# apache/horaedb

Hardware: NVIDIA H100
Metric: scanned rows/s (higher is better)
Workload: dtype f64

## Files before the change

### horaedb_b200/csrc/fused_scan.cu

```cuda
#include "fused_scan.h"

#include "block_scan.h"

#include <algorithm>
#include <cstddef>
#include <cstdlib>

namespace horae {
namespace fused {

namespace {

constexpr int MAXC = 8;
constexpr int kWarpsPerCta = 8;

struct alignas(16) FRec {
  uint32_t item, local;
  uint64_t gkey;
  int64_t bucket;
  uint64_t count;
  double sum, mn, mx;
  uint64_t _pad;
};

struct VSeg { const uint8_t* base1; uint32_t n0, _pad; };

enum : uint32_t { K_RAW64 = 0, K_U32 = 1, K_I32 = 2, K_F32 = 3 };
inline uint32_t kind_of(uint32_t t) {
  return (t == T_U64 || t == T_I64 || t == T_F64) ? K_RAW64 : (t == T_F32 ? K_F32 : ((t == T_I8 || t == T_I16 || t == T_I32) ? K_I32 : K_U32));
}
constexpr uint64_t kI32KeyLo = (1ull << 63) - (1ull << 31), kI32KeyHi = (1ull << 63) + (1ull << 31) - 1;

struct FParams {
  const SstDev* ssts;
  const RgSel* sel;
  const uint32_t* d_nsel;
  const uint8_t* const* bases;
  uint32_t split;
  uint32_t pcol[MAX_PREDS], pcls[MAX_PREDS];
  uint32_t pbloom[MAX_PREDS];
  uint64_t phash[MAX_PREDS];
  int nslots;
  uint32_t col[MAXC], kind[MAXC], cls[MAXC];
  int npk;
  int has_group, has_ts, value_slot, global_mode;
  int hot_slot[kHot];
  uint64_t hot_flip[kHot], hot_lo[kHot], hot_span[kHot];
  int hot_haspred[kHot];
  int npred;
  int pslot[MAX_PREDS];
  uint32_t pop[MAX_PREDS];
  uint64_t plit[MAX_PREDS];
  int64_t window_ms;
  const uint8_t* scratch;
  uint64_t scratch_stride;
  int region[MAXC];
  int value_stored;
  int gate_bits;
  int gate_slot;
  uint64_t bits_off;
  VSeg* vseg;
  FRec* rec;
  uint32_t rec_cap;
  uint32_t* item_cnt;
  unsigned int* work;
  unsigned long long* counters;
  int* err;
};

__device__ __forceinline__ uint64_t ld_bytes8(const uint8_t* p) {
  uintptr_t a = reinterpret_cast<uintptr_t>(p);
  uint32_t sh = uint32_t(a & 7) * 8;
  const uint64_t* q = reinterpret_cast<const uint64_t*>(a & ~uintptr_t(7));
  uint64_t lo = __ldg(q), hi = __ldg(q + 1);
  return (lo >> sh) | ((hi << 1) << (63 - sh));
}
__device__ __forceinline__ uint32_t ld32u(const uint8_t* p) { return uint32_t(ld_bytes8(p)); }

__device__ __forceinline__ uint64_t widen_kind(uint64_t raw, uint32_t kind) {
  uint32_t r = uint32_t(raw);
  uint64_t v = raw;
  v = kind == K_U32 ? uint64_t(r) : v;
  v = kind == K_I32 ? uint64_t(int64_t(int32_t(r))) : v;
  v = kind == K_F32 ? uint64_t(__double_as_longlong(double(__uint_as_float(r)))) : v;
  return v;
}
__device__ __forceinline__ uint64_t load_kind(const uint8_t* base, uint32_t kind, uint32_t row) {
  return widen_kind(ld_bytes8(base + size_t(row) * (kind == K_RAW64 ? 8u : 4u)), kind);
}

__device__ __forceinline__ uint32_t literal_header(const uint8_t* p, uint32_t* len) {
  const uint32_t t = __ldg(p);
  uint32_t l = t >> 2, hdr = 1;
  if (l >= 60) {
    const uint32_t nb = l - 59;
    l = 0;
    for (uint32_t i = 0; i < nb; i++) l |= uint32_t(__ldg(p + 1 + i)) << (8 * i);
    hdr = 1 + nb;
  }
  *len = l + 1;
  return hdr;
}

__device__ __forceinline__ const uint8_t* slot_base_chase(const FParams& P, uint32_t si, int s) {
  RgSel rs = P.sel[si];
  SstDev sst = P.ssts[rs.sst];
  ChunkDev cd = sst.chunks[size_t(rs.rg) * sst.ncols + P.col[s]];
  PageDev pg = sst.pages[cd.first_page];
  const uint8_t* body = sst.bytes + pg.payload_off;
  const bool is_value = P.value_stored && s == P.value_slot;
  if (cd.codec == 1) {
    if (is_value && cd.stored) {
      const uint8_t* p = body;
      while (__ldg(p) & 0x80) p++;
      p++;
      uint32_t len0 = 0, len1 = 0;
      const uint32_t h0 = literal_header(p, &len0);
      const uint8_t* lit0 = p + h0;
      const uint32_t prefix = cd.optional ? 4 + ld32u(lit0) : 0;
      const uint32_t w = P.kind[s] == K_RAW64 ? 8u : 4u;
      VSeg v;
      v.n0 = (len0 - prefix) / w;
      v._pad = 0;
      v.base1 = lit0 + prefix;
      if (lit0 + len0 < body + pg.comp_size) v.base1 = lit0 + len0 + literal_header(lit0 + len0, &len1);
      P.vseg[si] = v;
      return lit0 + prefix;
    }
    body = P.scratch + rs.scratch_off + uint64_t(P.region[s]) * P.scratch_stride;
  }
  if (cd.optional && s != P.gate_slot) {
    uint32_t lv = ld32u(body);
    if (lv > pg.uncomp_size) { lv = 0; atomicExch(P.err, 202); }
    body += 4 + lv;
  }
  if (is_value) { VSeg v; v.base1 = body; v.n0 = rs.num_rows; v._pad = 0; P.vseg[si] = v; }
  return body;
}
__device__ __forceinline__ const uint8_t* slot_base(const FParams& P, uint32_t si, int s) { return P.bases[size_t(si) * MAXC + s]; }
__device__ __noinline__ uint64_t fetch_val(const FParams& P, uint32_t si, int s, uint32_t row) {
  return load_kind(slot_base(P, si, s), P.kind[s], row);
}

struct Bucket { int64_t start, lo, hi; };
__device__ __noinline__ Bucket bucket_range(int64_t ts, int64_t w) {
  constexpr int64_t kMin = INT64_MIN, kMax = INT64_MAX;
  const int64_t r = w - 1;
  Bucket b;
  b.start = ts / w * w;
  if (b.start > 0) { b.lo = b.start; b.hi = b.start > kMax - r ? kMax : b.start + r; }
  else if (b.start < 0) { b.lo = b.start < kMin + r ? kMin : b.start - r; b.hi = b.start; }
  else { b.lo = -r; b.hi = r; }
  return b;
}

__device__ __noinline__ bool later_alive_dup(const FParams& P, uint32_t si, uint32_t row) {
  uint64_t pk[MAX_PK];
  for (int k = 0; k < P.npk; k++) pk[k] = fetch_val(P, si, k, row);
  uint32_t nrows = P.sel[si].num_rows;
  uint32_t r = row + 1;
  for (;;) {
    if (r >= nrows) {
      si++;
      if (si >= *P.d_nsel) return false;
      nrows = P.sel[si].num_rows;
      r = 0;
      if (nrows == 0) continue;
    }
    for (int k = 0; k < P.npk; k++)
      if (fetch_val(P, si, k, r) != pk[k]) return false;
    bool ok = true;
    if (P.gate_slot >= 0) {
      const uint32_t* gb = reinterpret_cast<const uint32_t*>(P.scratch + P.sel[si].scratch_off + P.bits_off);
      ok = (gb[r >> 5] >> (r & 31)) & 1u;
    }
    for (int p = 0; p < P.npred && ok; p++)
      if (P.pslot[p] != P.gate_slot) ok = op_holds(cmp_widened(fetch_val(P, si, P.pslot[p], r), P.plit[p], P.cls[P.pslot[p]]), P.pop[p]);
    if (ok) return true;
    r++;
  }
}

__device__ __forceinline__ uint64_t shfl64(uint64_t v, int src) {
  uint32_t lo = __shfl_sync(0xffffffffu, uint32_t(v), src);
  uint32_t hi = __shfl_sync(0xffffffffu, uint32_t(v >> 32), src);
  return (uint64_t(hi) << 32) | lo;
}
__device__ __forceinline__ double shfl_xor_d(double v, int m) {
  uint64_t b = uint64_t(__double_as_longlong(v));
  uint32_t lo = __shfl_xor_sync(0xffffffffu, uint32_t(b), m);
  uint32_t hi = __shfl_xor_sync(0xffffffffu, uint32_t(b >> 32), m);
  return __longlong_as_double((long long)((uint64_t(hi) << 32) | lo));
}

struct Acc {
  bool open;
  uint64_t g;
  int64_t bstart, blo, bhi;
  uint64_t cnt;
  double sum, mn, mx;
};

__device__ __noinline__ void emit(const FParams& P, const Acc& a, uint32_t item, uint32_t local, uint32_t* slots) {
  if (slots[0] == slots[1]) { slots[0] = atomicAdd(&P.work[1], 32u); slots[1] = slots[0] + 32u; }
  unsigned int slot = slots[0]++;
  if (slot < P.rec_cap) {
    FRec r;
    r.item = item; r.local = local; r.gkey = a.g; r.bucket = a.bstart; r.count = a.cnt; r.sum = a.sum; r.mn = a.mn; r.mx = a.mx; r._pad = 0;
    P.rec[slot] = r;
  } else atomicExch(P.err, 201);
}

struct FileDev {
  const RgCol* rgcol;
  const uint32_t* rg_rows;
  uint32_t rg_base, nrg, ncols, _pad;
  const uint8_t* bytes;
};

__global__ void __launch_bounds__(256) slot_bases_kernel(const __grid_constant__ FParams P, const uint8_t** __restrict__ bases) {
  const uint32_t idx = blockIdx.x * blockDim.x + threadIdx.x;
  const uint32_t si = idx / MAXC;
  const int s = int(idx % MAXC);
  if (si >= *P.d_nsel || s >= P.nslots) return;
  bases[idx] = slot_base_chase(P, si, s);
}

template <bool W4>
__global__ void __launch_bounds__(256, 8) gate_rg_kernel(const __grid_constant__ FParams P, RgSel* __restrict__ sel, int gate_slot, uint64_t flip,
                                                      uint64_t lo, uint64_t span, uint8_t* __restrict__ flags) {
  constexpr int kRows = W4 ? 8 : 4;
  __shared__ uint32_t s_last;
  __shared__ const uint8_t* s_base[256];
  const uint32_t nsel = *P.d_nsel;
  const int lane = threadIdx.x & 31;
  for (uint32_t k0 = 0; blockIdx.x + k0 * gridDim.x < nsel; k0 += 256) {
    {
      const uint32_t si = blockIdx.x + (k0 + threadIdx.x) * gridDim.x;
      if (si < nsel) s_base[threadIdx.x] = slot_base_chase(P, si, gate_slot);
    }
    for (uint32_t k = 0; k < 256; k++) {
      const uint32_t si = blockIdx.x + (k0 + k) * gridDim.x;
      if (si >= nsel) break;
      if (threadIdx.x == 0) s_last = 0;
      __syncthreads();
      const uint8_t* base = s_base[k];
      const RgSel rs = sel[si];
      const uint32_t nrows = rs.num_rows;
      uint32_t* bits = P.gate_bits ? reinterpret_cast<uint32_t*>(const_cast<uint8_t*>(P.scratch) + rs.scratch_off + P.bits_off) : nullptr;
      const bool aligned = (reinterpret_cast<uintptr_t>(base) & (W4 ? 3 : 7)) == 0;
      uint32_t last = 0;
      const uint32_t nw = (nrows + 31) >> 5;
      for (uint32_t i0 = 0; i0 < nw * 32; i0 += kRows * 256) {
        uint64_t v[kRows];
#pragma unroll
        for (int u = 0; u < kRows; u++) {
          const uint32_t i = i0 + u * 256 + threadIdx.x;
          v[u] = 0;
          if (i < nrows) {
            if (W4) v[u] = aligned ? __ldg(reinterpret_cast<const uint32_t*>(base) + i) : ld32u(base + size_t(i) * 4);
            else v[u] = aligned ? __ldg(reinterpret_cast<const unsigned long long*>(base) + i) : ld_bytes8(base + size_t(i) * 8);
          }
        }
#pragma unroll
        for (int u = 0; u < kRows; u++) {
          const uint32_t i = i0 + u * 256 + threadIdx.x;
          const bool pass = i < nrows && (W4 ? (uint32_t(v[u]) ^ uint32_t(flip)) - uint32_t(lo) <= uint32_t(span) : (v[u] ^ flip) - lo <= span);
          if (pass) last = i + 1;
          const uint32_t b = __ballot_sync(0xffffffffu, pass);
          if (bits && lane == 0 && (i >> 5) < nw) bits[i >> 5] = b;
        }
      }
      for (int d = 16; d > 0; d >>= 1) { const uint32_t o = __shfl_down_sync(0xffffffffu, last, d); last = o > last ? o : last; }
      if (lane == 0 && last) atomicMax(&s_last, last);
      __syncthreads();
      if (threadIdx.x == 0) {
        const uint32_t l = s_last;
        flags[si] = l ? 1 : 0;
        sel[si].out_row = l ? (l + 1 < nrows ? l + 1 : nrows) : 0;
      }
    }
    __syncthreads();
  }
}

__global__ void __launch_bounds__(1024) compact_sel_kernel(const RgSel* __restrict__ in, const uint8_t* __restrict__ flags, uint32_t* d_nsel,
                                                           RgSel* __restrict__ out, uint32_t* __restrict__ lpt) {
  __shared__ uint32_t s_w[1024 / 32 + 1];
  __shared__ uint32_t s_bin[1024];
  __shared__ uint32_t s_max;
  const uint32_t n = *d_nsel;
  const uint32_t per = (n + 1023u) / 1024u;
  const uint32_t lo = threadIdx.x * per;
  const uint32_t hi = lo + per < n ? lo + per : n;
  uint32_t cnt = 0;
  for (uint32_t i = lo; i < hi; i++) cnt += flags[i] != 0;
  s_bin[threadIdx.x] = 0;
  if (threadIdx.x == 0) s_max = 0;
  uint32_t m;
  uint32_t pos = block_excl_scan<1024>(cnt, &m, s_w);
  uint32_t mx = 0;
  for (uint32_t i = lo; i < hi; i++)
    if (flags[i]) { out[pos++] = in[i]; mx = in[i].out_row > mx ? in[i].out_row : mx; }
  if (lpt) {
    if (mx) atomicMax(&s_max, mx);
    __syncthreads();
    int shift = 0;
    while ((s_max >> shift) > 1023u) shift++;
    const uint32_t per2 = (m + 1023u) / 1024u;
    const uint32_t lo2 = threadIdx.x * per2, hi2 = lo2 + per2 < m ? lo2 + per2 : m;
    for (uint32_t i = lo2; i < hi2; i++) atomicAdd(&s_bin[1023u - (out[i].out_row >> shift)], 1u);
    __syncthreads();
    uint32_t nbin;
    const uint32_t start = block_excl_scan<1024>(s_bin[threadIdx.x], &nbin, s_w);
    s_bin[threadIdx.x] = start;
    __syncthreads();
    for (uint32_t i = lo2; i < hi2; i++) lpt[atomicAdd(&s_bin[1023u - (out[i].out_row >> shift)], 1u)] = i;
  }
  __syncthreads();
  if (threadIdx.x == 0) *d_nsel = m;
}

__global__ void __launch_bounds__(256) prune_rgs_kernel(const __grid_constant__ FParams P, const FileDev* __restrict__ files, int nfiles,
                                                        uint32_t total_rgs, int prune, uint32_t* __restrict__ keep_rows) {
  const uint32_t idx = blockIdx.x * blockDim.x + threadIdx.x;
  if (idx >= total_rgs) return;
  uint32_t f = 0;
  while (f + 1 < uint32_t(nfiles) && idx >= files[f + 1].rg_base) f++;
  const FileDev fd = files[f];
  const uint32_t rg = idx - fd.rg_base;
  const uint32_t rows = fd.rg_rows[rg];
  uint32_t keep = rows > 0;
  if (keep && prune) {
    const RgCol* rc = fd.rgcol + size_t(rg) * fd.ncols;
    for (int p = 0; p < P.npred && keep; p++) {
      const RgCol c = rc[P.pcol[p]];
      if (c.null_all) { keep = 0; break; }
      if (c.has_minmax && !minmax_may_match(c.mn, c.mx, P.plit[p], P.pop[p], P.pcls[p])) keep = 0;
      else if ((prune & 2) && P.pbloom[p] && c.bloom_blocks && !bloom::may_contain(fd.bytes + c.bloom_off, c.bloom_blocks, P.phash[p])) keep = 0;
    }
  }
  keep_rows[idx] = keep ? rows : 0;
}

__global__ void __launch_bounds__(1024) select_rgs_kernel(const FileDev* __restrict__ files, int nfiles, uint32_t total_rgs,
                                                          const uint32_t* keep_rows, RgSel* __restrict__ sel, uint32_t* d_nsel,
                                                          unsigned long long* counters, uint32_t smem_words, uint64_t scratch_per_rg) {
  extern __shared__ uint32_t s_keep[];
  __shared__ uint32_t s_w[1024 / 32 + 1];
  if (smem_words) {
    for (uint32_t i = threadIdx.x; i < total_rgs; i += 1024) s_keep[i] = keep_rows[i];
    __syncthreads();
    keep_rows = s_keep;
  }
  const uint32_t per = (total_rgs + 1023u) / 1024u;
  const uint32_t lo = threadIdx.x * per;
  const uint32_t hi = lo + per < total_rgs ? lo + per : total_rgs;
  uint32_t cnt = 0;
  unsigned long long rows_sel = 0;
  for (uint32_t i = lo; i < hi; i++) { const uint32_t r = keep_rows[i]; cnt += r > 0; rows_sel += r; }
  uint32_t nsel;
  uint32_t pos = block_excl_scan<1024>(cnt, &nsel, s_w);
  if (cnt) {
    uint32_t f = 0;
    for (uint32_t i = lo; i < hi; i++) {
      const uint32_t rows = keep_rows[i];
      if (rows == 0) continue;
      while (f + 1 < uint32_t(nfiles) && i >= files[f + 1].rg_base) f++;
      RgSel r;
      r.sst = f; r.rg = i - files[f].rg_base; r.out_row = 0; r.num_rows = rows; r.scratch_off = uint64_t(pos) * scratch_per_rg;
      sel[pos++] = r;
    }
  }
  for (int d = 16; d > 0; d >>= 1) rows_sel += __shfl_down_sync(0xffffffffu, rows_sel, d);
  if ((threadIdx.x & 31) == 0 && rows_sel) atomicAdd(&counters[2], rows_sel);
  if (threadIdx.x == 0) *d_nsel = nsel;
}

struct KeyRef { uint64_t g; int64_t lo, hi; };

__device__ __forceinline__ uint64_t pack_pos(uint32_t si, uint32_t row) { return (uint64_t(si) << 32) | row; }

template <bool HAS_TS>
struct BoundSearch {
  uint32_t j, si, row, L, H, ans;
  KeyRef k;
  const uint8_t *b0, *b1;
  bool done, found;

  __device__ __forceinline__ void finish(uint64_t* adj, uint64_t v, int lane) { if (lane == 0) adj[j] = v; done = true; }

  __device__ __forceinline__ void open_rg(const FParams& P) {
    b0 = P.has_group ? slot_base(P, si, 0) : nullptr;
    b1 = HAS_TS ? slot_base(P, si, 1) : nullptr;
    L = row;
    H = P.sel[si].num_rows;
    found = false;
    ans = H;
  }

  __device__ __forceinline__ void init(const FParams& P, uint32_t jj, uint32_t nsel, uint32_t nitems, uint64_t* adj, int lane) {
    j = jj;
    done = false;
    if (j > nitems) { done = true; return; }
    if (j == nitems) { finish(adj, pack_pos(nsel, 0), lane); return; }
    si = j / P.split;
    const uint32_t w = j % P.split;
    const uint32_t n = P.sel[si].num_rows;
    const uint32_t sr = (((n + P.split - 1) / P.split) + 31u) & ~31u;
    row = w * sr;
    if (row >= n) { si++; row = 0; }
    if (si >= nsel) { finish(adj, pack_pos(nsel, 0), lane); return; }
    if (P.global_mode || (si == 0 && row == 0)) { finish(adj, pack_pos(si, row), lane); return; }
    uint32_t psi = si, prow = row;
    if (prow == 0) { psi--; prow = P.sel[psi].num_rows - 1; } else prow--;
    k.g = P.has_group ? fetch_val(P, psi, 0, prow) : 0;
    k.lo = 0; k.hi = 0;
    if (HAS_TS) { Bucket b = bucket_range(int64_t(fetch_val(P, psi, 1, prow)), P.window_ms); k.lo = b.lo; k.hi = b.hi; }
    open_rg(P);
  }

  __device__ __forceinline__ uint32_t probe_pos(int lane, uint32_t* step) const {
    const uint32_t span = H - L;
    *step = (span + 31) / 32;
    uint32_t p = L + (uint32_t(lane) + 1) * *step - 1;
    return p >= H ? H - 1 : p;
  }

  __device__ __forceinline__ void advance(const FParams& P, unsigned m, uint32_t step, uint32_t nsel, uint64_t* adj, int lane) {
    if (m == 0) L = H;
    else {
      const int f = __ffs(m) - 1;
      uint32_t pf = L + (uint32_t(f) + 1) * step - 1;
      if (pf >= H) pf = H - 1;
      found = true;
      ans = pf;
      if (step == 1) L = H;
      else { L = L + uint32_t(f) * step; H = pf; }
    }
    if (L >= H) {
      if (found) { finish(adj, pack_pos(si, ans), lane); return; }
      si++;
      row = 0;
      if (si >= nsel) { finish(adj, pack_pos(nsel, 0), lane); return; }
      open_rg(P);
    }
  }
};

constexpr int kBoundsPerWarp = 4;

template <bool HAS_TS>
__global__ void __launch_bounds__(256) item_bounds_kernel(const __grid_constant__ FParams P, uint64_t* __restrict__ adj) {
  const int lane = threadIdx.x & 31;
  const uint32_t nsel = *P.d_nsel;
  const uint32_t nitems = nsel * P.split;
  const uint32_t warp = (blockIdx.x * blockDim.x + threadIdx.x) >> 5;
  BoundSearch<HAS_TS> bs[kBoundsPerWarp];
#pragma unroll
  for (int i = 0; i < kBoundsPerWarp; i++) bs[i].init(P, warp * kBoundsPerWarp + i, nsel, nitems, adj, lane);
  for (;;) {
    bool any = false;
    uint32_t step[kBoundsPerWarp];
    uint64_t v0[kBoundsPerWarp], v1[kBoundsPerWarp];
#pragma unroll
    for (int i = 0; i < kBoundsPerWarp; i++) {
      v0[i] = 0; v1[i] = 0; step[i] = 1;
      if (!bs[i].done) {
        any = true;
        const uint32_t p = bs[i].probe_pos(lane, &step[i]);
        if (P.has_group) v0[i] = load_kind(bs[i].b0, P.kind[0], p);
        if (HAS_TS) v1[i] = load_kind(bs[i].b1, P.kind[1], p);
      }
    }
    if (!any) break;
#pragma unroll
    for (int i = 0; i < kBoundsPerWarp; i++) {
      if (!bs[i].done) {
        bool ne = (P.has_group && v0[i] != bs[i].k.g) || (HAS_TS && (int64_t(v1[i]) < bs[i].k.lo || int64_t(v1[i]) > bs[i].k.hi));
        const unsigned m = __ballot_sync(0xffffffffu, ne);
        bs[i].advance(P, m, step[i], nsel, adj, lane);
      }
    }
  }
}

__device__ __forceinline__ double seq_sum_slice(double sum, unsigned keep_mask, bool keep, double v, double* s_vals, int lane) {
  if (__popc(keep_mask) >= 8) {
    __syncwarp();
    s_vals[lane] = keep ? v : 0.0;
    __syncwarp();
#pragma unroll
    for (int l = 0; l < 32; l++) sum += s_vals[l];
    return sum;
  }
  uint64_t vb = uint64_t(__double_as_longlong(v));
  while (keep_mask) {
    int l = __ffs(keep_mask) - 1;
    keep_mask &= keep_mask - 1;
    sum += __longlong_as_double((long long)shfl64(vb, l));
  }
  return sum;
}

template <bool HAS_TS>
__device__ __noinline__ void walk_slice(const FParams& P, Acc& acc, uint32_t& local, uint32_t item, unsigned keep_mask, bool keep, uint64_t g,
                                        int64_t ts, double v, double* s_vals, uint32_t* slots, int lane) {
  const double kInf = __longlong_as_double(0x7ff0000000000000LL);
  const bool has_val = P.value_slot >= 0;
  bool ext = keep && acc.open && (!P.has_group || g == acc.g) && (!HAS_TS || (ts >= acc.blo && ts <= acc.bhi));
  if (__ballot_sync(0xffffffffu, ext) == keep_mask) {
    acc.cnt += __popc(keep_mask);
    if (has_val) {
      const bool num = keep && v == v;
      double mn = num ? v : kInf, mx = num ? v : -kInf;
#pragma unroll
      for (int m = 1; m < 32; m <<= 1) {
        const double a = shfl_xor_d(mn, m), b = shfl_xor_d(mx, m);
        const bool later = (lane & m) != 0;
        mn = (later ? a <= mn : a < mn) ? a : mn;
        mx = (later ? b >= mx : b > mx) ? b : mx;
      }
      acc.mn = mn < acc.mn ? mn : acc.mn;
      acc.mx = mx > acc.mx ? mx : acc.mx;
      acc.sum = seq_sum_slice(acc.sum, keep_mask, keep, v, s_vals, lane);
    }
    return;
  }
  uint64_t vb = uint64_t(__double_as_longlong(v));
  while (keep_mask) {
    int l = __ffs(keep_mask) - 1;
    keep_mask &= keep_mask - 1;
    uint64_t kg = P.has_group ? shfl64(g, l) : 0;
    int64_t kt = HAS_TS ? int64_t(shfl64(uint64_t(ts), l)) : 0;
    if (!acc.open || kg != acc.g || (HAS_TS && (kt < acc.blo || kt > acc.bhi))) {
      if (acc.open) { if (lane == 0) emit(P, acc, item, local, slots); local++; }
      acc.open = true; acc.g = kg; acc.cnt = 0; acc.sum = 0.0; acc.mn = kInf; acc.mx = -kInf;
      if (HAS_TS) { Bucket b = bucket_range(kt, P.window_ms); acc.bstart = b.start; acc.blo = b.lo; acc.bhi = b.hi; }
      else { acc.bstart = 0; acc.blo = 0; acc.bhi = 0; }
    }
    acc.cnt++;
    if (has_val) {
      double x = __longlong_as_double((long long)shfl64(vb, l));
      acc.sum += x;
      if (acc.cnt == 1 || x < acc.mn) acc.mn = x;
      if (acc.cnt == 1 || x > acc.mx) acc.mx = x;
    }
  }
}

__device__ __forceinline__ double to_double_kind(uint64_t raw, uint32_t kind, uint32_t cls) {
  uint64_t wv = widen_kind(raw, kind);
  return cls == C_FLOAT ? __longlong_as_double((long long)wv) : (cls == C_SIGNED ? double(int64_t(wv)) : double(wv));
}

__device__ __forceinline__ uint64_t ld8(const uint8_t* q, uint32_t sh, uint32_t i) {
  const uint64_t* p = reinterpret_cast<const uint64_t*>(q) + i;
  uint64_t lo = __ldg(p), hi = __ldg(p + 1);
  uint32_t w0 = uint32_t(lo), w1 = uint32_t(lo >> 32), w2 = uint32_t(hi), w3 = uint32_t(hi >> 32);
  const bool up = (sh & 32u) != 0;
  const uint32_t s = sh & 31u;
  uint32_t a = up ? w1 : w0, b = up ? w2 : w1, c = up ? w3 : w2;
  return (uint64_t(__funnelshift_r(b, c, s)) << 32) | __funnelshift_r(a, b, s);
}
__device__ __forceinline__ uint32_t ld4(const uint8_t* q, uint32_t sh, uint32_t i) {
  const uint32_t* p = reinterpret_cast<const uint32_t*>(q) + i;
  uint32_t lo = __ldg(p), hi = __ldg(p + 1);
  return __funnelshift_r(lo, hi, sh);
// ... 648 lines not shown
  CU_TRY(d_sel.alloc(size_t(total_rgs + 1) * sizeof(RgSel), s));
  CU_TRY(d_keep.alloc(size_t(total_rgs + 1) * sizeof(uint32_t), s));
  CU_TRY(d_bsum.alloc(1024 * sizeof(uint32_t), s));
  CU_TRY(d_bases.alloc(size_t(total_rgs + 1) * MAXC * sizeof(uint8_t*), s));
  if (value_stored) CU_TRY(d_vseg.alloc(size_t(total_rgs + 1) * sizeof(VSeg), s));
  if (need_snappy()) {
    CU_TRY(d_sel2.alloc(size_t(total_rgs + 1) * sizeof(RgSel), s));
    CU_TRY(d_gflags.alloc(size_t(total_rgs) + 16, s));
    CU_TRY(d_lpt.alloc(size_t(total_rgs + 1) * sizeof(uint32_t), s));
    CU_TRY(d_scratch.alloc(size_t(total_rgs) * size_t(scratch_per_rg) + 256, s));
  }
  CU_TRY(out->alloc(bound, s));
  return HG_OK;
}

int FusedPlan::make_params() {
  std::vector<SstDev> sd(files.size());
  std::vector<FileDev> fdv(files.size());
  uint32_t rgb = 0;
  for (size_t i = 0; i < files.size(); i++) {
    SstResident* f = files[i];
    sd[i] = SstDev{f->d_bytes, f->d_pages, f->d_chunks, uint32_t(f->meta.ncols), uint32_t(f->meta.rgs.size())};
    fdv[i] = FileDev{f->d_rgcol, f->d_rg_rows, rgb, uint32_t(f->rg_rows.size()), uint32_t(f->meta.ncols), 0, f->d_bytes};
    rgb += uint32_t(f->rg_rows.size());
  }
  CU_TRY(d_ssts.alloc(sd.size() * sizeof(SstDev), e->stream));
  CU_TRY(d_files.alloc(fdv.size() * sizeof(FileDev), e->stream));
  int urc = stage_upload(e, d_ssts.p, sd.data(), sd.size() * sizeof(SstDev));
  if (!urc) urc = stage_upload(e, d_files.p, fdv.data(), fdv.size() * sizeof(FileDev));
  if (urc) return urc;

  std::memset(&P, 0, sizeof(P));
  P.ssts = d_ssts.as<SstDev>();
  P.sel = d_sel.as<RgSel>();
  P.d_nsel = &work->nsel;
  P.bases = d_bases.as<const uint8_t*>();
  P.split = split;
  P.nslots = int(S.slots.size());
  for (size_t i = 0; i < S.slots.size(); i++) {
    uint32_t t = schema->types[S.slots[i]];
    P.col[i] = S.slots[i];
    P.kind[i] = kind_of(t);
    P.cls[i] = cmp_class(t);
  }
  P.npk = int(schema->num_primary_keys);
  P.has_group = S.has_group;
  P.has_ts = S.has_ts;
  P.value_slot = S.value_slot;
  P.global_mode = S.global_mode;
  set_hot_params();
  P.npred = int(np);
  for (size_t i = 0; i < np; i++) {
    const uint32_t t = schema->types[preds[i].column];
    P.pslot[i] = S.pslot[i];
    P.pop[i] = preds[i].op;
    P.plit[i] = pred_literal(preds[i], t);
    P.pcol[i] = preds[i].column;
    P.pcls[i] = cmp_class(t);
    P.pbloom[i] = preds[i].op == HG_OP_EQ && bloom_literal_hash(P.plit[i], t, &P.phash[i]) ? 1u : 0u;
  }
  P.window_ms = S.has_ts ? agg->window_ms : 1;
  P.scratch = d_scratch.as<uint8_t>();
  P.scratch_stride = scratch_stride;
  for (int i = 0; i < MAXC; i++) P.region[i] = i < int(S.slots.size()) ? region[i] : -1;
  P.value_stored = value_stored ? 1 : 0;
  P.vseg = d_vseg.as<VSeg>();
  P.rec = d_rec.as<FRec>();
  P.rec_cap = uint32_t(rec_cap);
  P.item_cnt = d_item.as<uint32_t>();
  P.work = &work->item_ticket;
  P.counters = work->counters;
  P.err = &work->err;
  gated = !(e->flags & HG_FLAG_NO_LATE_MATERIALIZATION) && P.hot_haspred[S.nhot - 1] != 0;
  gate_first = need_snappy() && gated && region[gate_slot()] >= 0;
  P.gate_bits = gate_first ? 1 : 0;
  const int gs = gate_slot();
  const bool runs = slot_comp[gs] * 2 < rows_in_files;
  P.gate_slot = gate_first && runs && P.kind[gs] != K_RAW64 && gs >= P.npk && gs != S.value_slot ? gs : -1;
  P.bits_off = uint64_t(nregions) * scratch_stride;
  return HG_OK;
}

void FusedPlan::set_hot_params() {
  for (int h = 0; h < kHot; h++) {
    const int sl = h < S.nhot ? S.hot_slot[h] : 0;
    const uint32_t t = schema->types[S.slots[sl]];
    const bool w8 = (t == T_U64 || t == T_I64 || t == T_F64);
    P.hot_slot[h] = sl;
    P.hot_haspred[h] = (h < S.nhot && (S.klo[h] != 0 || S.khi[h] != ~0ull)) ? 1 : 0;
    uint64_t lo = S.klo[h], hi = S.khi[h];
    if (w8) P.hot_flip[h] = order_flip(t);
    else if (type_is_signed(t)) {
      P.hot_flip[h] = 1ull << 31;
      lo = lo < kI32KeyLo ? 0 : lo - kI32KeyLo;
      hi = hi > kI32KeyHi ? 0xffffffffull : hi - kI32KeyLo;
    } else {
      P.hot_flip[h] = 0;
      hi = std::min<uint64_t>(hi, 0xffffffffull);
    }
    P.hot_lo[h] = lo;
    P.hot_span[h] = hi >= lo ? hi - lo : 0;
    if (h >= 2 && h < S.nhot && !w8) xmask |= 1 << (h - 2);
  }
}

k::SnappyJob FusedPlan::make_job(const std::vector<int>& job_slots, unsigned int* ticket) const {
  k::SnappyJob J;
  std::memset(&J, 0, sizeof(J));
  J.ssts = P.ssts; J.sel = P.sel; J.d_nsel = P.d_nsel; J.nsel = 0; J.ncols = int(job_slots.size());
  std::vector<int> ord(job_slots.size());
  for (size_t i = 0; i < ord.size(); i++) ord[i] = int(i);
  std::stable_sort(ord.begin(), ord.end(), [&](int a, int b) { return slot_comp[job_slots[a]] > slot_comp[job_slots[b]]; });
  for (size_t i = 0; i < job_slots.size(); i++) {
    J.col[i] = S.slots[job_slots[i]];
    J.region[i] = uint32_t(region[job_slots[i]]);
    J.order[i] = uint8_t(ord[i]);
    J.skip_stored[i] = (value_stored && job_slots[i] == S.value_slot) ? 1 : 0;
  }
  J.fixed_stride = scratch_stride; J.scratch = d_scratch.as<uint8_t>(); J.ticket = ticket; J.err = P.err;
  return J;
}

void FusedPlan::decompress(const Launch& L) {
  cudaStream_t s = e->stream;
  const int gs = gate_slot();
  std::vector<int> first, rest;
  for (int i = 0; i < int(S.slots.size()); i++) {
    if (region[i] < 0) continue;
    if (gate_first && i == gs) first.push_back(i); else rest.push_back(i);
  }
  if (!first.empty()) {
    const uint32_t gt = schema->types[S.slots[gs]];
    const bool w4 = !(gt == T_U64 || gt == T_I64 || gt == T_F64);
    const int h = S.nhot - 1;
    if (P.gate_slot >= 0) {
      k::GateJob G;
      G.J = make_job(first, &work->snappy_ticket[0]);
      G.sel = d_sel.as<RgSel>(); G.bits_off = P.bits_off;
      G.flip = uint32_t(P.hot_flip[h]); G.lo = uint32_t(P.hot_lo[h]); G.span = uint32_t(P.hot_span[h]);
      G.flags = d_gflags.as<uint8_t>(); G.fallback = &work->gate_fallback;
      k::snappy_gate_pages(L, G, total_rgs);
    } else {
      k::snappy_pages(L, make_job(first, &work->snappy_ticket[0]), total_rgs);
      if (w4) gate_rg_kernel<true><<<kNumSMs * 8, 256, 0, s>>>(P, d_sel.as<RgSel>(), gs, P.hot_flip[h], P.hot_lo[h], P.hot_span[h], d_gflags.as<uint8_t>());
      else gate_rg_kernel<false><<<kNumSMs * 8, 256, 0, s>>>(P, d_sel.as<RgSel>(), gs, P.hot_flip[h], P.hot_lo[h], P.hot_span[h], d_gflags.as<uint8_t>());
      L.tick();
    }
    compact_sel_kernel<<<1, 1024, 0, s>>>(d_sel.as<RgSel>(), d_gflags.as<uint8_t>(), &work->nsel, d_sel2.as<RgSel>(), d_lpt.as<uint32_t>());
    L.tick();
    P.sel = d_sel2.as<RgSel>();
  }
  if (!rest.empty()) {
    k::SnappyJob J2 = make_job(rest, &work->snappy_ticket[1]);
    if (!first.empty() && !S.has_ts)
      for (size_t i = 0; i < rest.size(); i++) J2.partial[i] = rest[i] != 0 ? 1 : 0;
    if (!first.empty()) { J2.sel = P.sel; J2.lpt = d_lpt.as<uint32_t>(); }
    k::snappy_pages(L, J2, total_rgs * uint32_t(rest.size()));
  }
}

int FusedPlan::launch() {
  cudaStream_t s = e->stream;
  Launch L = e->L();
  const FileDev* fd = d_files.as<FileDev>();
  prune_rgs_kernel<<<(total_rgs + 255) / 256, 256, 0, s>>>(P, fd, int(files.size()), total_rgs,
                                                           (e->flags & HG_FLAG_NO_PRUNING) ? 0 : ((e->flags & HG_FLAG_NO_BLOOM_FILTER) ? 1 : 3),
                                                           d_keep.as<uint32_t>());
  L.tick();
  CU_TRY(cudaFuncSetAttribute(select_rgs_kernel, cudaFuncAttributeMaxDynamicSharedMemorySize, 200 * 1024));
  const uint32_t smem_words = size_t(total_rgs) * 4 <= 200 * 1024 ? total_rgs : 0;
  select_rgs_kernel<<<1, 1024, size_t(smem_words) * 4, s>>>(fd, int(files.size()), total_rgs, d_keep.as<uint32_t>(), d_sel.as<RgSel>(),
                                                            &work->nsel, work->counters, smem_words, scratch_per_rg);
  L.tick();
  CU_TRY(cudaEventRecord(e->evd0, s));
  if (need_snappy()) decompress(L);
  CU_TRY(cudaEventRecord(e->evd1, s));
  slot_bases_kernel<<<(total_rgs * MAXC + 255) / 256, 256, 0, s>>>(P, d_bases.as<const uint8_t*>());
  L.tick();
  const uint32_t nb = (nitems + 1 + kBoundsPerWarp - 1) / kBoundsPerWarp;
  const int bctas = int((uint64_t(nb) * 32 + 255) / 256);
  if (S.has_ts) item_bounds_kernel<true><<<bctas, 256, 0, s>>>(P, d_adj.as<uint64_t>());
  else item_bounds_kernel<false><<<bctas, 256, 0, s>>>(P, d_adj.as<uint64_t>());
  L.tick();
  CU_TRY(cudaEventRecord(e->evk0, s));
  const int ctas = int(std::min<uint64_t>((uint64_t(nitems) + kWarpsPerCta - 1) / kWarpsPerCta, uint64_t(kNumSMs) * 8));
  launch_fused<2, 4>(S.nhot, xmask, S.has_ts, gated, ctas, s, P, d_adj.as<uint64_t>());
  L.tick();
  CU_TRY(cudaEventRecord(e->evk1, s));
  if (S.global_mode) {
    global_count_kernel<<<1, 1, 0, s>>>(work->counters, out->out());
    L.tick();
  } else {
    const uint32_t sblocks = (nitems + 1023) / 1024;
    item_scan_kernel<<<sblocks, 1024, 0, s>>>(d_item.as<uint32_t>(), &work->nsel, split, d_bsum.as<uint32_t>());
    L.tick();
    scatter_records_kernel<<<kNumSMs * 4, 256, 0, s>>>(d_rec.as<FRec>(), &work->rec_slots, d_item.as<uint32_t>(), d_bsum.as<uint32_t>(), sblocks,
                                                       &work->groups, out->gwidth, out->out(), uint32_t(std::min<uint64_t>(bound, 0xffffffffu)),
                                                       uint32_t(std::min<uint64_t>(rec_cap, 0xffffffffu)), &work->err);
    L.tick();
  }
  return HG_OK;
}

int FusedPlan::read_back() {
  WorkBlock w;
  std::memset(&w, 0, sizeof(w));
  if (total_rgs > 0) {
    const auto t3 = HostClock::now();
    if (!e->h_small) CU_TRY(cudaMallocHost(&e->h_small, 256));
    CU_TRY(cudaMemcpyAsync(e->h_small, work, sizeof(WorkBlock), cudaMemcpyDeviceToHost, e->stream));
    CU_TRY(cudaStreamSynchronize(e->stream));
    std::memcpy(&w, e->h_small, sizeof(w));
    const auto t4 = HostClock::now();
    if (trace_on())
      fprintf(stderr, "[fused] plan %.0f us, bound+alloc %.0f us, upload+launch %.0f us, wait %.0f us (row groups %u, max items %u, gate chunks decompressed %u)\n",
              elapsed_us(t0, t1), elapsed_us(t1, t2), elapsed_us(t2, t3), elapsed_us(t3, t4), total_rgs, nitems, w.gate_fallback);
    if (w.err >= 201 && w.err <= 203)
      return set_error(HG_ERR_FORMAT, "fused scan: rows contradict their chunk statistics or a page is damaged (device error " + std::to_string(w.err) + ")");
    if (w.err) return set_error(HG_ERR_INTERNAL, "fused scan: device error " + std::to_string(w.err));
    float kms = 0;
    cudaEventElapsedTime(&kms, e->evk0, e->evk1);
    e->stats.kernel_ms = kms;
    if (need_snappy()) { cudaEventElapsedTime(&kms, e->evd0, e->evd1); e->stats.decomp_ms = kms; }
  }
  out->G = S.global_mode ? (w.counters[1] > 0 ? 1u : 0u) : w.groups;
  e->stats.rows_in_files = rows_in_files;
  e->stats.rows_decoded = w.counters[2];
  e->stats.rows_materialized = w.counters[3];
  e->stats.rows_filtered = w.counters[0];
  e->stats.rows_out = w.counters[1];
  e->stats.groups_out = out->G;
  e->stats.path = 1;
  return HG_OK;
}

}

int try_scan_aggregate(hg_engine* e, const hg_schema_desc* schema, const hg_sst_desc* ssts, size_t n, const hg_predicate* preds,
                       size_t np, const hg_agg_spec* agg, AggBuffers* out) {
  FusedPlan F{e, schema, preds, np, agg, out};
  if (fused_shape(schema, preds, np, agg, &F.S) == NOT_APPLICABLE) return NOT_APPLICABLE;
  F.t0 = HostClock::now();
  int rc = F.plan_files(ssts, n);
  if (rc) return rc;
  out->gtype = F.S.has_group ? schema->types[0] : uint32_t(T_U64);
  out->gwidth = F.S.has_group ? type_width(out->gtype) : 8;
  if (F.S.empty_interval) return F.empty_answer();
  F.lay_out_scratch();
  F.t1 = HostClock::now();
  if ((rc = F.size_groups()) || (rc = F.alloc())) return rc;
  F.t2 = HostClock::now();
  if (F.total_rgs > 0 && ((rc = F.make_params()) || (rc = F.launch()))) return rc;
  return F.read_back();
}


}
}
```

### horaedb_b200/csrc/snappy_core.h

```cpp
#pragma once
#include <cstdint>

#ifndef SNP_STAT
#define SNP_STAT(counter, amount)
#endif
#ifndef SNP_STAT_VALUE
#define SNP_STAT_VALUE(amount)
#endif

namespace horae {
namespace snp {

constexpr int kWin = 256;
constexpr int kWinPad = 16;
constexpr int kRing = 4096;
constexpr int kHist = 2048;
constexpr int kLevels = 6;
constexpr int kMinValues = 8;
constexpr uint32_t kExit = 0xff;
constexpr uint32_t kRestage = kWin - 80;
constexpr uint32_t kFlushAt = 512;
constexpr uint64_t kFill = 0xfcfcfcfcfcfcfcfcull;

constexpr int kStage = 448;
// ... 338 lines not shown
            const uint32_t l1 = (s >> 5) & 7u, l2 = (t >> 5) & 7u;
            const uint32_t mine = uint32_t((1ull << (8 * l1)) - 1);
            s = (t & 31u) | ((l1 > l2 ? l1 : l2) << 5) | (((s & mine) | (t & ~mine)) & 0xffffff00u);
          }
          const uint32_t lk = (s >> 5) & 7u;
          const uint64_t root = shfl64(w, int(s & 31u));
          const uint64_t v = (root & (~0ull << (8 * lk))) | (s & 0xffffff00u) | (lit4 & 0xffu);
          const uint32_t wb = o >> 3;
          if (!ph) {
            if (in) sm.ring64[(wb + uint32_t(lane)) & (kRing / 8 - 1)] = v;
          } else {
            const uint32_t sh = 8 * ph;
            uint64_t prev = (uint64_t(snp_shfl_up(uint32_t(v >> 32), 1)) << 32) | snp_shfl_up(uint32_t(v), 1);
            uint64_t lo = prev >> (64 - sh);
            if (lane == 0) lo = sm.ring64[wb & (kRing / 8 - 1)] & ((1ull << sh) - 1);
            if (in) sm.ring64[(wb + uint32_t(lane)) & (kRing / 8 - 1)] = lo | (v << sh);
            if (lane == cv - 1) sm.ring64[(wb + uint32_t(lane) + 1) & (kRing / 8 - 1)] = v >> (64 - sh);
          }
          snp_syncwarp();
          const uint32_t T = uint32_t(cv) * 8;
          SNP_STAT(steps, 1); SNP_STAT_VALUE(1); SNP_STAT(elements, 2 * cv); SNP_STAT(bytes, T);
          first = false;
          o += T;
          if (o - fl >= kFlushAt) fl = flush_words(sm, dst, fl, o, lane);
          const uint32_t adv = snp_shfl(qc + ccsz, cv - 1);
          if (adv > kRestage || adv >= avail || o >= stop_at) { pos += adv; break; }
          qs = adv;
          snp_syncwarp();
          continue;
        }
      }
      uint32_t q = qs;
#pragma unroll
      for (int lv = 0; lv < 5; lv++)
        if ((lane >> lv) & 1) q = sm.J[lv][q];
      const uint32_t e = lut[sm8[wbase + q]];
      uint32_t len = e & 0x7fu;
      uint32_t ecsz = e >> 24;
      bool is_lit = (e >> 16) & 1u;
      uint32_t off;
      {
        const uint32_t p1 = wbase + q + 1;
        const uint32_t raw = snp_funnel_r(sm32[p1 >> 2], sm32[(p1 >> 2) + 1], (p1 & 3) * 8);
        off = is_lit ? 0u : ((raw & (0xffffffffu >> ((e >> 18) & 31u))) | (e & 0x700u));
      }
      const bool valid = q != kExit && !((e >> 17) & 1u) && q + ecsz <= avail;
      const unsigned vm = snp_ballot(valid);
      const int m = (vm == 0xffffffffu) ? 32 : (snp_ffs(~vm) - 1);
      if (m == 0) {
        if (first) { if (lane == 0) snp_set_err(err, 105); return; }
        pos += qs;
        break;
      }
      first = false;
      if (lane >= m) { len = 0; ecsz = 0; off = 1; is_lit = true; }
      uint32_t inc = len;
#pragma unroll
      for (int d = 1; d < 32; d <<= 1) { const uint32_t t = snp_shfl_up(inc, d); if (lane >= d) inc += t; }
      const uint32_t doff = inc - len;
      {
        const bool bad = lane < m && !is_lit && (off == 0 || off > o + doff);
        if (snp_any(bad)) { if (lane == 0) snp_set_err(err, 103); return; }
      }
      const uint32_t len0 = snp_shfl(len, 0);
      int cnt;
      uint32_t T;
      if (len0 <= 8) {
        uint32_t skind = 0, spos = 0;
        bool fail = len > 8;
        const uint32_t s0 = doff - off;
        if (!is_lit && !fail) {
          if (off >= len) {
            if (s0 + len - 1 >= 0x80000000u) { skind = 1; spos = o + s0; }
            else if (s0 >= 0x80000000u) fail = true;
            else skind = 2;
          } else {
            if (doff == 0) { skind = 1; spos = o - off; } else fail = true;
          }
        }
        uint64_t w = 0;
        if (lane < m && !fail && skind != 2) {
          const uint32_t r = spos & (kRing - 1);
          if (skind == 1 && o - spos > uint32_t(kHist)) w = ld8_out(dst + spos);
          else if (skind == 1 && r > uint32_t(kRing) - 8) w = ring_ld8(sm, spos);
          else w = sm_ld8(sm, skind == 0 ? wbase + q + 1 : r);
          if (skind == 1 && off < len) {
            w &= (off >= 8) ? ~0ull : ((1ull << (8 * off)) - 1);
            for (uint32_t f = off; f < 8; f <<= 1) w |= w << (8 * f);
          }
        }
        uint32_t pp = uint32_t(lane);
        bool need = false;
        {
          const int cand = lane - int(off >> 2);
          const uint32_t x = snp_shfl(doff | (len << 16), cand);
          if (skind == 2) {
            const uint32_t d = s0 - (x & 0xffffu);
            if (cand >= 0 && cand < lane && d < 0x10000u && d + len <= (x >> 16)) pp = uint32_t(cand) | (d << 8);
            else need = true;
          }
        }
        if (snp_any(need)) {
          SNP_STAT(parent_searches, 1);
          int lo = 0;
#pragma unroll
          for (int step = 16; step > 0; step >>= 1) {
            const int cand = lo + step;
            const uint32_t d = snp_shfl(doff, cand & 31);
            if (need && cand < lane && d <= s0) lo = cand;
          }
          const uint32_t pd = snp_shfl(doff, lo), pl = snp_shfl(len, lo);
          if (need) {
            if (lo >= lane || s0 < pd || s0 + len > pd + pl) fail = true;
            else pp = uint32_t(lo) | ((s0 - pd) << 8);
          }
        }
        const unsigned fm = snp_ballot(fail || lane >= m);
        cnt = fm ? snp_ffs(fm) - 1 : 32;
        if (vmode) {
          const uint32_t nx = snp_shfl(len | (uint32_t(!is_lit && off != 0 && !(off & 7u)) << 8), (lane + 1) & 31);
          const bool pair = lane < 31 && is_lit && len <= 4u && nx == (8u - len) + 0x100u;
          const bool cand = pair && 2 * lane >= cnt && lane < cnt;
          const unsigned pm = snp_ballot(cand);
          const unsigned last = snp_ballot(cand && (pm >> lane) == 1u);
          if (last) cnt = snp_ffs(last) - 1;
        }
        if (lane >= cnt) pp = uint32_t(lane);
#pragma unroll
        for (int it = 0; it < 5; it++) pp = snp_shfl(pp, int(pp)) + (pp & ~0xffu);
        {
          const uint64_t wr = shfl64(w, int(pp));
          if (skind == 2) w = wr >> (8 * (pp >> 8));
        }
        T = snp_shfl(inc, cnt - 1);
        if (o + T > ulen) { if (lane == 0) snp_set_err(err, 103); return; }
        if (lane < cnt) {
          const uint32_t rb = (o + doff) & (kRing - 1);
          if (rb <= uint32_t(kRing) - 8) store_elem(sm, smbase, rb, w, len);
          else {
#pragma unroll
            for (int i = 0; i < 8; i++)
              if (uint32_t(i) < len) ring[(rb + i) & (kRing - 1)] = uint8_t(w >> (8 * i));
          }
        }
      } else {
        const uint32_t off0 = snp_shfl(off, 0);
        const bool lit0 = snp_shfl(uint32_t(is_lit), 0) != 0;
        if (lit0) cnt = 1;
        else {
          const unsigned brk = snp_ballot(lane >= m || is_lit || off != off0);
          cnt = brk ? snp_ffs(brk) - 1 : 32;
        }
        T = snp_shfl(inc, cnt - 1);
        if (o + T > ulen) { if (lane == 0) snp_set_err(err, 103); return; }
        snp_syncwarp();
        if (lit0) {
          const uint32_t q0 = snp_shfl(q, 0);
          const uint8_t* ls = src + pos + q0 + 1;
          for (uint32_t i = lane; i < T; i += 32) ring[(o + i) & (kRing - 1)] = snp_ldg8(ls + i);
        } else if (off0 == 8 || off0 == 4 || off0 == 2 || off0 == 1) {
          uint64_t pw = ring_ld8(sm, o - off0);
          pw &= (off0 >= 8) ? ~0ull : ((1ull << (8 * off0)) - 1);
          for (uint32_t f = off0; f < 8; f <<= 1) pw |= pw << (8 * f);
          const uint32_t c = (off0 - (o % off0)) % off0;
          const uint64_t W = c ? ((pw >> (8 * c)) | (pw << (64 - 8 * c))) : pw;
          const uint32_t a0 = (o + 7) & ~7u, a1 = (o + T) & ~7u;
          if (a0 < a1) {
            for (uint32_t wd = (a0 >> 3) + lane; wd < (a1 >> 3); wd += 32) sm.ring64[wd & (kRing / 8 - 1)] = W;
            if (o + lane < a0) ring[(o + lane) & (kRing - 1)] = uint8_t(W >> (8 * ((o + lane) & 7)));
            if (a1 + lane < o + T) ring[(a1 + lane) & (kRing - 1)] = uint8_t(W >> (8 * lane));
          } else {
            for (uint32_t i = o + lane; i < o + T; i += 32) ring[i & (kRing - 1)] = uint8_t(W >> (8 * (i & 7)));
          }
        } else {
          const uint32_t stride = 32u % off0;
          uint32_t r = uint32_t(lane) % off0;
          for (uint32_t i = lane; i < T; i += 32) {
            const uint32_t x = o - off0 + r;
            ring[(o + i) & (kRing - 1)] = old_byte(sm, dst, o, x);
            r += stride;
            if (r >= off0) r -= off0;
          }
        }
      }
      snp_syncwarp();
      SNP_STAT(steps, 1); SNP_STAT(elements, cnt); SNP_STAT(word_steps, len0 <= 8 ? 1 : 0); SNP_STAT(bytes, T);
      o += T;
      if (o - fl >= kFlushAt) fl = flush_words(sm, dst, fl, o, lane);
      const uint32_t adv = snp_shfl(q + ecsz, cnt - 1);
      if (adv > kRestage || adv >= avail || o >= stop_at) { pos += adv; break; }
      qs = adv;
      snp_syncwarp();
    }
  }
  snp_syncwarp();
  fl = flush_words(sm, dst, fl, o, lane);
  if (fl + lane < o) dst[fl + lane] = ring[(fl + lane) & (kRing - 1)];
  if (o != ulen && o < stop_at) { if (lane == 0) snp_set_err(err, 104); }
}

SNP_FN void snappy_page(const uint8_t* __restrict__ src, uint32_t n, uint8_t* __restrict__ dst, uint32_t ulen_expected, uint32_t stop_at,
                        WarpSmem& sm, uint32_t& phase, const uint8_t* __restrict__ csz, const uint32_t* __restrict__ lut, int lane, int* err,
                        bool vmode = false) {
  StageState st;
  st.phase = phase; st.cur = 0; st.pf = false; st.pf_start = 0; st.pf_bytes = 0;
  snappy_page_body(src, n, dst, ulen_expected, stop_at, vmode, sm, st, csz, lut, lane, err);
  snp_syncwarp();
  if (st.pf) {
    const int nb = st.cur ^ 1;
    bulk_wait(sm, nb, (st.phase >> nb) & 1u);
    st.phase ^= 1u << nb;
  }
  phase = st.phase;
}

constexpr int kGateCap = 256;
constexpr int kGateRows = 8192;
constexpr int kGateHops = 16;
constexpr uint32_t kGateLit = 0x80000000u;
#ifdef __CUDACC__
#define SNP_POPC(x) __popc(x)
#define SNP_CLZ(x) __clz(x)
#else
#define SNP_POPC(x) __builtin_popcount(x)
#define SNP_CLZ(x) __builtin_clz(x)
#endif
struct GateTab {
  uint32_t d[kGateCap];
  uint32_t len[kGateCap];
  uint32_t src[kGateCap];
  uint32_t bits[kGateRows / 32];
};
static_assert(sizeof(GateTab) <= sizeof(WarpSmem::ring64), "the gate decoder's tables live in the ring");
struct GateTest { uint32_t flip, lo, span; };
SNP_FN bool gate_pass(const GateTest& g, uint32_t v) { return (v ^ g.flip) - g.lo <= g.span; }

SNP_FN bool gate_byte(const GateTab& t, uint32_t ntab, const uint8_t* __restrict__ src, uint32_t y, uint32_t& out) {
  for (int h = 0; h < kGateHops; h++) {
    uint32_t i = 0;
    for (uint32_t step = kGateCap / 2; step; step >>= 1)
      if (i + step < ntab && t.d[i + step] <= y) i += step;
    const uint32_t s = t.src[i], d = t.d[i];
    if (s & kGateLit) { out = snp_ldg8(src + (s & ~kGateLit) + (y - d)); return true; }
    y = (y - d >= s) ? d - s + (y - d) % s : y - s;
  }
  return false;
}
SNP_FN uint32_t gate_get32(const GateTab& t, uint32_t r) {
  const uint32_t w = r >> 5, sh = r & 31;
  if (!sh) return t.bits[w];
  return snp_funnel_r(t.bits[w], w + 1 < uint32_t(kGateRows / 32) ? t.bits[w + 1] : 0u, sh);
}
SNP_FN void gate_or(GateTab& t, uint32_t v, uint32_t m) {
  if (!m) return;
  const uint32_t w = v >> 5, sh = v & 31;
  t.bits[w] |= m << sh;
  if (sh && (m >> (32 - sh))) t.bits[w + 1] |= m >> (32 - sh);
}
SNP_FN bool gate_resolve(GateTab& t, uint32_t ntab, const uint8_t* __restrict__ src, uint32_t P, uint32_t va, uint32_t vb, const GateTest& g,
                         int lane) {
  bool ok = true;
  for (uint32_t v0 = va; v0 < vb; v0 += 8) {
    const uint32_t v = v0 + uint32_t(lane >> 2);
    uint32_t b = 0;
    if (v < vb && !gate_byte(t, ntab, src, P + 4 * v + uint32_t(lane & 3), b)) ok = false;
    const uint32_t b1 = snp_shfl(b, (lane + 1) & 31), b2 = snp_shfl(b, (lane + 2) & 31), b3 = snp_shfl(b, (lane + 3) & 31);
    const bool pass = v < vb && !(lane & 3) && gate_pass(g, b | (b1 << 8) | (b2 << 16) | (b3 << 24));
    const uint32_t m = snp_ballot(pass);
    uint32_t m8 = 0;
#pragma unroll
    for (int k = 0; k < 8; k++) m8 |= ((m >> (4 * k)) & 1u) << k;
    if (lane == 0) gate_or(t, v0, m8);
    snp_syncwarp();
  }
  return !snp_any(!ok);
}
SNP_FN void gate_literal(GateTab& t, const uint8_t* __restrict__ src, uint32_t P, uint32_t d, uint32_t sp, uint32_t va, uint32_t vb,
                         const GateTest& g, int lane) {
  for (uint32_t v0 = va; v0 < vb; v0 += 32) {
    const uint32_t v = v0 + uint32_t(lane);
    bool pass = false;
    if (v < vb) {
      const uint8_t* p = src + sp + (P + 4 * v - d);
      pass = gate_pass(g, uint32_t(snp_ldg8(p)) | (uint32_t(snp_ldg8(p + 1)) << 8) | (uint32_t(snp_ldg8(p + 2)) << 16) |
                              (uint32_t(snp_ldg8(p + 3)) << 24));
    }
    const uint32_t m = snp_ballot(pass);
    if (lane == 0) gate_or(t, v0, m);
    snp_syncwarp();
  }
}
SNP_FN void gate_fill(GateTab& t, uint32_t va, uint32_t vb, uint32_t p, int lane) {
  for (uint32_t w = (va >> 5) + uint32_t(lane); w < ((vb + 31) >> 5); w += 32) {
    const uint32_t x0 = w * 32 > va ? w * 32 : va, x1 = w * 32 + 32 < vb ? w * 32 + 32 : vb;
    const uint32_t r = (x0 - va) % p;
    uint32_t pat;
    if (p >= 32) {
      const uint32_t a = gate_get32(t, va - p + r);
      pat = p - r >= 32 ? a : ((a & ((1u << (p - r)) - 1)) | (gate_get32(t, va - p) << (p - r)));
    } else {
      const uint64_t pm = (1ull << p) - 1, base = gate_get32(t, va - p) & pm;
      uint64_t y = ((base >> r) | (base << (p - r))) & pm;
      for (uint32_t l = p; l < 32; l <<= 1) y |= y << l;
      pat = uint32_t(y);
    }
    const uint32_t n = x1 - x0;
// ... 170 lines not shown
```

Measured before the change: 56.12 billion.

## Extend repeated-copy runs in snappy decoder and bound scans to gated live rows

The snappy decoder now checks whether a full warp of identical short-offset copies repeats further in the compressed stream. It uses ballots to absorb many more repeated elements into a single run fill, cutting per-element decode iterations on highly repetitive pages. Separately, the scan and dedup code limit row ranges to the gated live-row count (out_row) when gate bits are active. All rest-column pages are marked partial when a gating first pass exists, so fewer rows are decoded. This adds extra lookahead work and a flush per extension, and the change in row bounds alters semantics that must stay consistent with compaction.

```diff
diff --git a/horaedb_b200/csrc/fused_scan.cu b/horaedb_b200/csrc/fused_scan.cu
--- a/horaedb_b200/csrc/fused_scan.cu
+++ b/horaedb_b200/csrc/fused_scan.cu
@@ -138,6 +138,10 @@
   return body;
 }
 __device__ __forceinline__ const uint8_t* slot_base(const FParams& P, uint32_t si, int s) { return P.bases[size_t(si) * MAXC + s]; }
+__device__ __forceinline__ uint32_t live_rows(const FParams& P, uint32_t si) {
+  const RgSel& rs = P.sel[si];
+  return P.gate_bits ? rs.out_row : rs.num_rows;
+}
 __device__ __noinline__ uint64_t fetch_val(const FParams& P, uint32_t si, int s, uint32_t row) {
   return load_kind(slot_base(P, si, s), P.kind[s], row);
 }
@@ -157,13 +161,13 @@
 __device__ __noinline__ bool later_alive_dup(const FParams& P, uint32_t si, uint32_t row) {
   uint64_t pk[MAX_PK];
   for (int k = 0; k < P.npk; k++) pk[k] = fetch_val(P, si, k, row);
-  uint32_t nrows = P.sel[si].num_rows;
+  uint32_t nrows = live_rows(P, si);
   uint32_t r = row + 1;
   for (;;) {
     if (r >= nrows) {
       si++;
       if (si >= *P.d_nsel) return false;
-      nrows = P.sel[si].num_rows;
+      nrows = live_rows(P, si);
       r = 0;
       if (nrows == 0) continue;
     }
@@ -394,7 +398,7 @@
     b0 = P.has_group ? slot_base(P, si, 0) : nullptr;
     b1 = HAS_TS ? slot_base(P, si, 1) : nullptr;
     L = row;
-    H = P.sel[si].num_rows;
+    H = live_rows(P, si);
     found = false;
     ans = H;
   }
@@ -406,14 +410,14 @@
     if (j == nitems) { finish(adj, pack_pos(nsel, 0), lane); return; }
     si = j / P.split;
     const uint32_t w = j % P.split;
-    const uint32_t n = P.sel[si].num_rows;
+    const uint32_t n = live_rows(P, si);
     const uint32_t sr = (((n + P.split - 1) / P.split) + 31u) & ~31u;
     row = w * sr;
     if (row >= n) { si++; row = 0; }
     if (si >= nsel) { finish(adj, pack_pos(nsel, 0), lane); return; }
     if (P.global_mode || (si == 0 && row == 0)) { finish(adj, pack_pos(si, row), lane); return; }
     uint32_t psi = si, prow = row;
-    if (prow == 0) { psi--; prow = P.sel[psi].num_rows - 1; } else prow--;
+    if (prow == 0) { psi--; prow = live_rows(P, psi) - 1; } else prow--;
     k.g = P.has_group ? fetch_val(P, psi, 0, prow) : 0;
     k.lo = 0; k.hi = 0;
     if (HAS_TS) { Bucket b = bucket_range(int64_t(fetch_val(P, psi, 1, prow)), P.window_ms); k.lo = b.lo; k.hi = b.hi; }
@@ -1368,8 +1372,8 @@
   }
   if (!rest.empty()) {
     k::SnappyJob J2 = make_job(rest, &work->snappy_ticket[1]);
-    if (!first.empty() && !S.has_ts)
-      for (size_t i = 0; i < rest.size(); i++) J2.partial[i] = rest[i] != 0 ? 1 : 0;
+    if (!first.empty())
+      for (size_t i = 0; i < rest.size(); i++) J2.partial[i] = 1;
     if (!first.empty()) { J2.sel = P.sel; J2.lpt = d_lpt.as<uint32_t>(); }
     k::snappy_pages(L, J2, total_rgs * uint32_t(rest.size()));
   }
diff --git a/horaedb_b200/csrc/snappy_core.h b/horaedb_b200/csrc/snappy_core.h
--- a/horaedb_b200/csrc/snappy_core.h
+++ b/horaedb_b200/csrc/snappy_core.h
@@ -514,6 +514,39 @@
           cnt = brk ? snp_ffs(brk) - 1 : 32;
         }
         T = snp_shfl(inc, cnt - 1);
+        const bool word_run = off0 == 8 || off0 == 4 || off0 == 2 || off0 == 1;
+        if (cnt == 32 && word_run && o + T < stop_at) {
+          const uint32_t q31 = snp_shfl(q, 31), c = snp_shfl(ecsz, 31), l31 = snp_shfl(len, 31);
+          const uint32_t lim = avail < uint32_t(kWin + kWinPad) ? avail : uint32_t(kWin + kWinPad);
+          uint32_t maxext = (uint32_t(kRing) - 32u - T) / l31;
+          const uint32_t need = (stop_at - o - T) / l31 + 1;
+          if (need < maxext) maxext = need;
+          const uint32_t a = wbase + q31;
+          const uint32_t ref = snp_funnel_r(sm32[a >> 2], sm32[(a >> 2) + 1], (a & 3) * 8);
+          const uint32_t mask = c >= 4 ? 0xffffffffu : (1u << (8 * c)) - 1;
+          uint32_t ext = 0;
+          for (;;) {
+            const uint32_t pj = q31 + c * (1 + ext + uint32_t(lane));
+            bool same = ext + uint32_t(lane) < maxext && pj + c <= lim;
+            if (same) {
+              const uint32_t b = wbase + pj;
+              const uint32_t x = snp_funnel_r(sm32[b >> 2], sm32[(b >> 2) + 1], (b & 3) * 8);
+              same = ((x ^ ref) & mask) == 0 && (c < 5 || sm8[a + 4] == sm8[b + 4]);
+            }
+            const unsigned sm_same = snp_ballot(same);
+            const uint32_t k = sm_same == 0xffffffffu ? 32u : uint32_t(snp_ffs(~sm_same) - 1);
+            ext += k;
+            if (k < 32) break;
+          }
+          if (ext) {
+            snp_syncwarp();
+            fl = flush_words(sm, dst, fl, o, lane);
+            snp_syncwarp();
+            T += ext * l31;
+            SNP_STAT(elements, ext);
+            if (lane == 31) ecsz += ext * c;
+          }
+        }
         if (o + T > ulen) { if (lane == 0) snp_set_err(err, 103); return; }
         snp_syncwarp();
         if (lit0) {
```

After: 57.35 billion, median of 6. 1.02x the previous value.
